# JohnGBaker/ptmcmc

Hardware: AMD Instinct MI355X
Metric: ladder-wide MH steps/sec (D=32 Gaussian, 1024 temps) (higher is better)
Workload: dtype f64

## Files before the change

ptmcmc_amd/csrc/ptm_decide.hpp:

```cpp
#pragma once
#include "ptm_kernels.hpp"

namespace ptm {

constexpr int MSG_HDR = 2;
constexpr int ROW_EXTRA = 4;

__device__ __forceinline__ double* claim_row(double* buf, int cap, int RD, int* err) {
  const int slot = atomicAdd(reinterpret_cast<int*>(buf), 1);
  if (slot >= cap) { atomicOr(err, 4); return nullptr; }
  return buf + MSG_HDR + (size_t)slot * RD;
}

struct Decide {
  int DP, Nt, r0, nloc, W, Nc, ms;
  int w_off;
  uint64_t seed, step;
  double thresh;
  const double* beta;
  const double* ll_below;
  const double* ll_above;
  int H;
  const double* ll_all;
  const double* lp_all;
// ... 680 lines not shown
    d2_t v[NQ];
    const int msrc = lane < nmv ? gs[lane] : 0;
    const int dme = lane < nmv ? gd[lane] : -3;
    const double sl = dme >= 0 ? llc[p.r0 + dme / p.W] : p.ll[msrc];
    const double sp = p.lp_is_const ? p.lp_const : p.lp[msrc];
    for (int hc = 0; hc < DPm; hc += 32) {
      const int colh = col + hc;
#pragma unroll
      for (int q = 0; q < NQ; ++q) {
        const int j = GR * q + g;
        v[q] = *reinterpret_cast<const d2_t*>(p.x + (size_t)(j < nmv ? gs[j] : 0) * DPm + colh);
      }
      asm volatile("s_waitcnt vmcnt(0)" ::: "memory");
      __syncthreads();
#pragma unroll
      for (int q = 0; q < NQ; ++q) {
        const int j = GR * q + g;
        const int d = j < nmv ? gd[j] : -3;
        if (d != -3 && act) {
          double* dstp;
          if (d >= 0) dstp = p.x + (size_t)d * DPm;
          else if (d <= HIST_DST) {
            const int c = HIST_DST - d;
            dstp = p.hist.x + hist_slot(p.hist, 1 + (long long)(p.nhist[c] / (unsigned int)p.add_every_n), c) * DPm;
          } else if (d <= MAP_DST) {
            dstp = p.map.x + (size_t)(MAP_DST - d) * DPm;
          } else { const int e = -d - 4; dstp = ((e & 1) ? p.send_down : p.send_up) + MSG_HDR + (size_t)(e >> 1) * RD; }
          *reinterpret_cast<d2_t*>(dstp + colh) = v[q];
        }
      }
    }
    if (lane < nmv) {
      const int d = gd[lane];
      if (d >= 0) { p.ll[d] = sl; if (!p.lp_is_const) p.lp[d] = sp; }
      else if (d <= HIST_DST) {
        const int c = HIST_DST - d;
        const long long hrow = 1 + (long long)(p.nhist[c] / (unsigned int)p.add_every_n);
        hist_scalars(p.hist, hist_slot(p.hist, hrow, c), hrow, sl, sp, p.naccept[c], p.ntries[c], p.last_type[c],
                     evb ? gb[lane] : beta[p.r0 + c / p.W]);
      } else if (d <= MAP_DST) {
        const int c = MAP_DST - d;
        const double t = (evb ? gb[lane] : beta[p.r0 + c / p.W]) * sl;
        p.map.lpost[c] = sp + t; p.map.ll[c] = sl; p.map.lp[c] = sp;
      } else if (d != -3) {
        const int e = -d - 4;
        double* row = ((e & 1) ? p.send_down : p.send_up) + MSG_HDR + (size_t)(e >> 1) * RD;
        row[DPm] = sl; row[DPm + 1] = sp; row[DPm + 2] = (double)w; row[DPm + 3] = 0.0;
      }
    }
    return;
  }
  const int DP = p.DP;
  if (p.hist.rungs) {
    for (int j = lane; j < nl; j += DECIDE_THREADS) {
      const int k = list[j];
      if (alive[k] != 1) continue;
      const int i = cand[k];
      const int hs = hist_mid_src(i);
      if (hs < 0) continue;
      const int c = (i - p.r0) * p.W + w;
      const long long hrow = 1 + (long long)(p.nhist[c] / (unsigned int)p.add_every_n);
      const size_t o = hist_slot(p.hist, hrow, c);
      for (int d = 0; d < DP; ++d) p.hist.x[o * DP + d] = p.x[(size_t)hs * DP + d];
      hist_scalars(p.hist, o, hrow, p.ll[hs], p.lp[hs], p.naccept[c], p.ntries[c], p.last_type[c], evb ? bklo[k] : beta[i]);
    }
    __syncthreads();
  }
  if (p.map.rungs) {
    for (int j = lane; j < nl; j += DECIDE_THREADS) {
      const int k = list[j];
      if (alive[k] != 1) continue;
      const int i = cand[k];
      const double bmid = evb ? bklo[k] : beta[i];
      const int cs = map_mid_src(i, bmid);
      if (cs < 0) continue;
      const int c = (i - p.r0) * p.W + w;
      const double t = bmid * p.ll[cs];
      p.map.lpost[c] = p.lp[cs] + t; p.map.ll[c] = p.ll[cs]; p.map.lp[c] = p.lp[cs];
      for (int d = 0; d < DP; ++d) p.map.x[(size_t)c * DP + d] = p.x[(size_t)cs * DP + d];
    }
    __syncthreads();
  }
  for (int j = lane; j < nl; j += DECIDE_THREADS) {
    const int k = list[j];
    if (alive[k] != 1) continue;
    const int i = cand[k];
    const int rtop = (PTM_ALIVE_RUNG(i + 1) && alive[first[i + 1]] == 1) ? i : i + 1;
    for (int r = i; r <= rtop; ++r) {
      if (r < p.r0 || r >= r1 || perm[r] == r) continue;
      const int to = inv[r];
      const bool departs = to < p.r0 || to >= r1;
      bool head = departs;
      if (!departs) {
        head = true;
        int cc = perm[r], guard = 0;
        while (cc != r) {
          if (cc < p.r0 || cc >= r1 || cc < r || ++guard > Nt) { head = false; break; }
          cc = perm[cc];
        }
      }
      if (!head) continue;
      double* X = p.x;
      const int c0 = (r - p.r0) * p.W + w;
      if (departs) {
        double* sb = (to >= r1) ? p.send_up : p.send_down;
        if (!sb) continue;
        double* row = claim_row(sb, p.row_cap, DP + ROW_EXTRA, p.err);
        if (row) {
          for (int d = 0; d < DP; ++d) row[d] = X[(size_t)c0 * DP + d];
          row[DP] = p.ll[c0];
          row[DP + 1] = p.lp[c0];
          row[DP + 2] = (double)w;
          row[DP + 3] = 0.0;
        }
      }
      if (p.rowof) {
        const unsigned short carry = p.rowof[c0];
        int cur = r;
        for (int guard = 0; guard <= Nt; ++guard) {
          const int src = perm[cur];
          const int cc = (cur - p.r0) * p.W + w;
          if (src == r) { p.rowof[cc] = carry; break; }
          if (src < p.r0 || src >= r1) break;
          p.rowof[cc] = p.rowof[(src - p.r0) * p.W + w];
          cur = src;
        }
      }
      for (int el = p.rowof ? DP : 0; el < DP + 2; ++el) {
        auto at = [&](int c) -> double* { return el < DP ? X + (size_t)c * DP + el : (el == DP ? p.ll + c : p.lp + c); };
        const double carry = *at(c0);
        int cur = r;
        for (int guard = 0; guard <= Nt; ++guard) {
          const int src = perm[cur];
          const int cc = (cur - p.r0) * p.W + w;
          if (src == r) { *at(cc) = carry; break; }
          if (src < p.r0 || src >= r1) break;
          const int cs = (src - p.r0) * p.W + w;
          *at(cc) = *at(cs);
          cur = src;
        }
      }
    }
  }
  if (lane == 0) p.mv_n[w] = 0;
#undef PTM_ALIVE_RUNG
}

template <int DECIDE_THREADS, bool CUT = false>
__global__ __launch_bounds__(DECIDE_THREADS) void decide_kernel(const Decide p) {
  extern __shared__ __attribute__((aligned(16))) unsigned char smem[];
  decide_body<DECIDE_THREADS, CUT>(p, smem, xcd_walker(blockIdx.x, p.W), p.step, p.swap_log);
}

inline size_t decide_lds_bytes(int Nt, int ms, int WN, bool evolve, bool evb, bool cut = false) {
  if (cut) return decide_lds_bytes(Nt, ms, WN, evolve, true) + (size_t)2 * Nt * 8;
  const bool al = decide_aliased(ms, WN, evolve);
  const size_t msp = (size_t)((ms + 3) & ~3), WNp = (size_t)((WN + 3) & ~3);
  return (size_t)WN * 8 + (size_t)((Nt + 3) & ~3) * 2 + (size_t)((ms + 1) & ~1) * 4 * 2 + 16 + (al ? 0 : 2 * WNp * 2) + 2 * msp * 2 +
         (size_t)((ms + 7) & ~7) * 2 + (al ? 0 : (size_t)2 * MVCAP * 4) + 32 +
         (evolve ? ((size_t)Nt + 2 * ((Nt + 31) / 32) + 2 + 4 * msp) * 8 + 4 * msp * 2 + ((ms + 7) & ~7) : 0) +
         (evb ? ((size_t)(Nt > MVCAP ? Nt : MVCAP) + 5 * msp) * 8 : 0);
}


}
```

ptmcmc_amd/csrc/ptm_engine.hip:

```cpp
#include <hip/hip_runtime.h>

#include <algorithm>
#include <cmath>
#include <cstddef>
#include <cstdarg>
#include <cstdio>
#include <cstring>
#include <functional>
#include <memory>
#include <string>
#include <vector>

#include "../../include/ptm_engine.h"
#include "ptm_aux_kernels.hpp"
#include "ptm_devlike_kernels.hpp"
#include "ptm_ess_kernels.hpp"
#include "ptm_launch.hpp"
#include "ptm_shard_rccl.hpp"

using namespace ptm;

static thread_local std::string g_err;
static int fail(int code, const char* fmt, ...) {
  char buf[512];
// ... 1009 lines not shown
                                 "history_capacity that holds every row of the run");
  if (e->pcb) return fail(PTM_ERR_INVALID, "host-side proposals are set (ptm_set_proposal_callback): they replace every device proposal");
  if (!(q->snooker >= 0 && q->snooker <= 1) || !(q->gamma_one_frac >= 0 && q->gamma_one_frac <= 1) || !(q->reduce_gamma > 0) ||
      !(q->ignore_frac >= 0 && q->ignore_frac < 1) || n_init_extra < 0 || (n_init_extra > 0 && !init_rows))
    return fail(PTM_ERR_INVALID, "differential evolution: snooker and gamma_one_frac in [0, 1], reduce_gamma > 0, ignore_frac in [0, 1), init rows given");
  int rc;
  if (n_init_extra > 0) {
    const size_t Nc = e->Nc, D = e->D, DP = e->DP;
    std::vector<double> img((size_t)n_init_extra * Nc * DP, 0.0);
    for (size_t k = 0; k < (size_t)n_init_extra; ++k)
      for (size_t c = 0; c < Nc; ++c)
        for (size_t d = 0; d < D; ++d) img[(k * Nc + c) * DP + host_row_pos(DP, d)] = init_rows[(k * Nc + c) * D + d];
    if ((rc = dalloc(&e->de_init, img.size()))) return rc;
    HIPCHK(hipMemcpy(e->de_init, img.data(), img.size() * 8, hipMemcpyHostToDevice));
  }
  if (!e->de_hast && ((rc = dalloc(&e->de_hast, (size_t)e->Nc)) || (rc = dalloc(&e->de_type, (size_t)e->Nc)))) return rc;
  e->de = *q;
  e->de_init_extra = n_init_extra;
  e->de_on = true;
  return PTM_OK;
}

extern "C" int ptm_set_proposal_rung(ptm_engine* e, int local_rung, const double* factor, double one_d_frac) {
  SETTLE(e);
  if (!e || !factor) return fail(PTM_ERR_INVALID, "null argument");
  if (!e->have_prop) return fail(PTM_ERR_INVALID, "set all proposals first (ptm_set_proposals)");
  if (local_rung < 0 || local_rung >= e->nloc) return fail(PTM_ERR_INVALID, "rung out of the shard");
  const int D = e->D, DP = e->DP, kind = e->prop_kind == KIND_DIAG ? PTM_PROP_DIAG : (e->prop_kind == KIND_LOWER ? PTM_PROP_LOWER : PTM_PROP_DENSE);
  std::vector<double> packed((size_t)e->prop_stride, 0.0);
  if (kind == PTM_PROP_DIAG) {
    for (int d = 0; d < D; ++d) packed[d] = factor[d];
  } else {
    for (int i = 0; i < D; ++i)
      for (int j = 0; j < D; ++j) {
        if (kind == PTM_PROP_LOWER && j > i && factor[(size_t)i * D + j] != 0.0)
          return fail(PTM_ERR_INVALID, "PTM_PROP_LOWER factor has a non-zero above the diagonal");
        packed[(size_t)j * DP + i] = factor[(size_t)i * D + j];
      }
  }
  int rc;
  if ((rc = upload(e->prop + (size_t)local_rung * e->prop_stride, packed.data(), packed.size(), e->stream))) return rc;
  if (DP == 32) {
    std::vector<double> tiles(16 * 64, 0.0);
    for (int t = 0; t < 16; ++t) {
      const int rt = t & 1, sl = (t >> 1) & 3, hb = t >> 3;
      for (int k = 0; k < 4; ++k)
        for (int i = 0; i < 16; ++i) {
          const int row = 16 * rt + i, col = 16 * hb + 4 * k + sl;
          if (row < D && col < D)
            tiles[(size_t)t * 64 + 16 * k + i] = kind == PTM_PROP_DIAG ? (row == col ? factor[row] : 0.0) : factor[(size_t)row * D + col];
        }
    }
    if ((rc = upload(e->prop_tiles + (size_t)local_rung * 16 * 64, tiles.data(), tiles.size(), e->stream))) return rc;
  }
  if (DP == 64 || DP == 128) {
    const int NT = DP / 16, ntile = NT * NT * 4;
    std::vector<double> tiles((size_t)ntile * 64, 0.0);
    for (int t = 0; t < ntile; ++t) {
      const int rt = t % NT, sl = (t / NT) & 3, hb = t / (4 * NT);
      for (int k = 0; k < 4; ++k)
        for (int i = 0; i < 16; ++i) {
          const int row = 16 * rt + i, col = 16 * hb + 4 * k + sl;
          if (row < D && col < D)
            tiles[(size_t)t * 64 + 16 * k + i] = kind == PTM_PROP_DIAG ? (row == col ? factor[row] : 0.0) : factor[(size_t)row * D + col];
        }
    }
    if ((rc = upload(e->prop_tiles + (size_t)local_rung * ntile * 64, tiles.data(), tiles.size(), e->stream))) return rc;
  }
  if (one_d_frac >= 0) {
    if (one_d_frac > 1) return fail(PTM_ERR_INVALID, "oneDfrac must be in [0,1]");
    if ((rc = upload(e->onedfrac + local_rung, &one_d_frac, 1, e->stream))) return rc;
    if (one_d_frac > 0) e->any_oned = 1;
  }
  return PTM_OK;
}

static Dev make_dev(ptm_engine* e, bool labelled = false) {
  Dev p;
  memset(&p, 0, sizeof p);
  p.D = e->D; p.DP = e->DP; p.Nt = e->Nt; p.r0 = e->r0; p.nloc = e->nloc; p.W = e->W; p.Nc = e->Nc; p.w_off = e->cfg.walker_begin;
  p.seed = e->cfg.seed; p.step = e->step; p.add_every_n = e->cfg.add_every_n; p.min_prior = e->cfg.min_prior;
  p.has_bounds = e->has_bounds; p.origin_valid = e->origin_valid; p.bounds_box = e->bounds_box;
  p.blo = e->blo; p.bhi = e->bhi; p.bmin = e->bmin; p.bmax = e->bmax;
  p.all_uniform = e->all_uniform; p.lprior_const = e->lprior_const;
  p.ptype = e->ptype; p.plo = e->plo; p.phi = e->phi; p.pcoef = e->pcoef;
  p.P2 = e->P2; p.mean = e->mean; p.has_mean = e->has_mean; p.like0 = e->like0;
  p.beta = e->beta; p.prop = e->prop; p.prop_tiles = e->prop_tiles; p.P2_tiles = e->P2_tiles; p.box_row = e->box_row; p.onedfrac = e->onedfrac; p.prop_stride = e->prop_stride; p.any_oned = e->any_oned;
  p.mix_K = e->mix_K; p.mix = e->mix;
  p.de_on = e->de_on ? 1 : 0; p.de_init_extra = e->de_init_extra; p.de_init = e->de_init; p.de_hast = e->de_hast; p.de_type = e->de_type;
  p.de_snooker = e->de.snooker; p.de_gamma_one = e->de.gamma_one_frac; p.de_gamma_div = e->de.reduce_gamma; p.de_ignore = e->de.ignore_frac;
  p.de_gamma_std = e->de_on ? 1.68 / std::sqrt((double)e->D) / e->de.reduce_gamma : 0.0;
  p.betaC = e->betaC; p.beta_add = e->beta_add; p.beta_w = e->beta_w;
  p.x = labelled ? e->xdev : xrows(e); p.ll = e->ll; p.lp = e->lp;
  p.ntries = e->ntries; p.naccept = e->naccept; p.last_type = e->last_type; p.nhist = e->nhist;
  p.touch = e->touch; p.err = e->err;
  p.hist = e->hist;
  p.map = e->map;
  p.c_begin = 0; p.c_end = e->Nc;
  p.host_prop = e->pcb ? 1 : 0; p.hastings = e->hastings; p.htype = e->htype; p.hvalid = e->hvalid; p.acc_out = e->acc_out;
  return p;
}

static AdaArgs make_ada(const ptm_engine* e) {
  AdaArgs a;
  memset(&a, 0, sizeof a);
  if (!e->ada_on) return a;
  const size_t L = (size_t)e->ada.K + e->ada.K_inner, Nc = e->Nc;
  a.K = e->ada.K; a.nested = e->ada.nested; a.Ki = e->ada.K_inner; a.rate = e->ada.rate; a.rate_in = e->ada.rate_inner;
  a.leaf = e->ada_leaf; a.w = e->ada_dbl; a.th = e->ada_dbl + L * Nc; a.bits = e->ada_int; a.cnt = e->ada_int + 2 * Nc;
  return a;
}

static inline bool user_like(const ptm_engine* e) { return e->cb != nullptr || e->dfn != nullptr; }

static SweepSel sweep_sel(const ptm_engine* e) {
  SweepSel s;
  s.kind = e->prop_kind == PTM_PROP_DIAG ? KIND_DIAG : (e->prop_kind == PTM_PROP_LOWER ? KIND_LOWER : KIND_DENSE);
  s.uni = (e->W % 64) == 0;
  s.host_prop = e->pcb != nullptr;
  if (s.host_prop) s.kind = KIND_DIAG;
  s.ada = e->ada_on && !s.host_prop;
  s.plain = !e->has_bounds && e->all_uniform && !e->has_mean && !e->any_oned && !user_like(e) && e->mix_K == 0 && !s.ada && !e->betaC && !s.host_prop;
  s.simple = s.uni && s.plain;
  s.lean_ev = s.uni && e->betaC && !e->has_bounds && e->all_uniform && !e->has_mean && !e->any_oned && !user_like(e) && e->mix_K == 0 && !s.ada && !s.host_prop &&
              !e->hist.rungs && !e->map.rungs;
  s.callback = user_like(e);
  s.de = e->de_on;
  return s;
}

static bool lean_ev_sweeps(const ptm_engine* e) {
  static const bool forced = [] { const char* v = getenv("PTM_FORCE_VALU"); return v && *v && *v != '0'; }();
  return e->DP == 32 && !forced && sweep_sel(e).lean_ev;
}

static int flush_nhist(ptm_engine* e) {
  if (!e->nhist_pending) return PTM_OK;
  hipLaunchKernelGGL(nhist_flush_kernel, dim3((unsigned)(((size_t)e->Nc + 255) / 256)), dim3(256), 0, e->stream, e->nhist, (size_t)e->Nc, e->nhist_pending);
  HIPCHK(hipGetLastError());
  e->nhist_pending = 0;
  return PTM_OK;
}

static bool compact_applies(const ptm_engine* e, const SweepSel& sel) {
  static const bool compact_ok = [] { const char* v = getenv("PTM_COMPACT"); return !(v && *v == '0'); }();
  const bool gen1 = sel.uni && !sel.callback && !sel.host_prop && !sel.de && !sel.ada && e->all_uniform && (!e->has_bounds || e->bounds_box);
  return compact_ok && e->DP == 32 && (sel.simple || gen1) && !e->hist.rungs && !e->map.rungs && !getenv("PTM_FORCE_VALU") &&
         e->W >= 1024 && e->nloc <= 4096;
}
static bool row_labels_apply(const ptm_engine* e) {
  static const bool labels_ok = [] { const char* v = getenv("PTM_ROW_LABELS"); return !(v && *v == '0'); }();
  return labels_ok && e->nloc == e->Nt && !e->shard && e->W <= 65536 && e->Nt > 1 && compact_applies(e, sweep_sel(e));
}
static void flush_rows(ptm_engine* e) {
  e->rows_labelled = false;
  hipLaunchKernelGGL(restore_rows_kernel, dim3(e->W), dim3(256), (size_t)4 * e->nloc, e->stream, e->xdev, e->rowof, e->W, e->nloc, e->DP);
}

static int ensure_betaC(ptm_engine* e);
static int callback_host_part(ptm_engine* e) {
  const size_t Nc = e->Nc, DP = e->DP;
  HIPCHK(copy_unless_shared(e->h_xprop.data(), e->xprop, Nc * DP * 8 + Nc, hipMemcpyDeviceToHost, e->stream));
  HIPCHK(hipStreamSynchronize(e->stream));
  if (e->prior_cb) {
    std::vector<double> hll(Nc), hlp(Nc), hbeta(Nc), out;
    HIPCHK(hipMemcpy(hll.data(), e->ll, Nc * 8, hipMemcpyDeviceToHost));
    HIPCHK(hipMemcpy(hlp.data(), e->lp, Nc * 8, hipMemcpyDeviceToHost));
    { int rc2 = ensure_betaC(e); if (rc2) return rc2; }
    if (e->betaC) HIPCHK(hipMemcpy(hbeta.data(), e->betaC, Nc * 8, hipMemcpyDeviceToHost));
    std::vector<size_t> vp;
    for (size_t c = 0; c < Nc; ++c)
      if (e->h_gate[c] & 1) vp.push_back(c);
    int rcp = call_user_prior(e, e->h_xprop, vp, out);
    if (rcp) return rcp;
    std::vector<double> lpn(Nc, -__builtin_inf());
    for (size_t k = 0; k < vp.size(); ++k) {
      const size_t c = vp[k];
      const double beta = e->betaC ? hbeta[c] : e->h_beta[e->r0 + c / e->W];
      const double bl = beta * hll[c];
      const double cur_lpost = hlp[c] + bl;
      const double oldlprior = cur_lpost - bl;
      const double nl = out[k];
      lpn[c] = nl;
      const bool want = nl > -1e200 || nl - oldlprior > e->cfg.min_prior;
      e->h_gate[c] = (unsigned char)(1 | (want ? 2 : 0));
    }
    HIPCHK(hipMemcpyAsync(e->lprior_new, lpn.data(), Nc * 8, hipMemcpyHostToDevice, e->stream));
    HIPCHK(copy_unless_shared(e->gate, e->h_gate, Nc, hipMemcpyHostToDevice, e->stream));
    HIPCHK(hipStreamSynchronize(e->stream));
  }
  std::vector<size_t> pick;
  for (size_t c = 0; c < Nc; ++c)
    if (e->h_gate[c] & 2) pick.push_back(c);
  int rc = call_user(e, e->h_xprop, pick, e->h_llbatch);
  if (rc) return rc;
  for (size_t k = 0; k < pick.size(); ++k) e->h_llnew[pick[k]] = e->h_llbatch[k];
  HIPCHK(copy_unless_shared(e->llike_new, e->h_llnew.data(), Nc * 8, hipMemcpyHostToDevice, e->stream));
  return PTM_OK;
}

static int devlike_eval(ptm_engine* e, const unsigned char* gate, int gmask, int gval, const double* xsel, const double* xrest, double* dst,
                        unsigned char* gate_out, const double* lprior, bool best) {
  const int n = e->Nc, D = e->D;
  const int nchunk = (n + DL_CHUNK - 1) / DL_CHUNK;
  hipLaunchKernelGGL(devlike_count_kernel, dim3(nchunk), dim3(DL_CHUNK), 0, e->stream, n, gate, gmask, gval, e->dl_chunks);
  HIPCHK(hipGetLastError());
#define PTM_DL_PACK(N) case N: hipLaunchKernelGGL((devlike_pack_kernel<N>), dim3(nchunk), dim3(DL_CHUNK), 0, e->stream, n, D, nchunk, gate, gmask, gval, \
                                                  (const int*)e->dl_chunks, xsel, xrest, e->dl_x, e->dl_rows, e->dl_count); break;
  switch (e->DP) {
    PTM_DL_PACK(4) PTM_DL_PACK(8) PTM_DL_PACK(16) PTM_DL_PACK(32) PTM_DL_PACK(64) PTM_DL_PACK(128) PTM_DL_PACK(256) PTM_DL_PACK(512) PTM_DL_PACK(1024)
    default: return fail(PTM_ERR_UNSUPPORTED, "dim > 1024 is not built");
  }
#undef PTM_DL_PACK
  HIPCHK(hipGetLastError());
  if (!xrest) {
    const size_t tot = (size_t)n * D;
    hipLaunchKernelGGL(devlike_fill_kernel, dim3((unsigned)((tot + 255) / 256)), dim3(256), 0, e->stream, n, D, (const int32_t*)e->dl_count, e->dl_x);
    HIPCHK(hipGetLastError());
  }
  e->dfn(e->dfn_user, (void*)e->stream, n, D, e->dl_x, e->dl_count, e->dl_ll);
  hipLaunchKernelGGL(devlike_scatter_kernel, dim3(1), dim3(DL_SCATTER_THREADS), 0, e->stream, D, (const int32_t*)e->dl_count, (const int*)e->dl_rows,
                     (const double*)e->dl_ll, dst, gate_out, lprior, (const double*)e->dl_x, best ? e->dl_best : nullptr);
  HIPCHK(hipGetLastError());
  return PTM_OK;
}

static int devlike_reset_best(ptm_engine* e) {
  if (!e->dl_best) return PTM_OK;
  std::vector<double> b((size_t)e->D + 1, 0.0);
  b[0] = -__builtin_inf();
  return upload(e->dl_best, b.data(), b.size(), e->stream);
}

extern "C" int ptm_set_target_device(ptm_engine* e, ptm_loglike_device_fn fn, void* user, double* x_batch_dev, double* llike_batch_dev) {
  if (!e || !fn) return fail(PTM_ERR_INVALID, "null argument");
  SETTLE(e);
  NO_BATCH(e, "ptm_set_target_device");
  if (e->prior_cb) return fail(PTM_ERR_UNSUPPORTED, "a host-evaluated prior with a device likelihood is not built (ptm_set_prior_callback)");
  if (e->pcb) return fail(PTM_ERR_UNSUPPORTED, "host-side proposals with a device likelihood are not built (ptm_set_proposal_callback)");
  if (e->nloc != e->Nt) return fail(PTM_ERR_UNSUPPORTED, "a device likelihood on a rung shard is not built: split such a population by walkers");
  const size_t Nc = e->Nc, D = e->D, DP = e->DP;
  int rc;
  if (!e->dl_count &&
      ((rc = dalloc(&e->dl_count, 1)) || (rc = dalloc(&e->dl_rows, Nc)) || (rc = dalloc(&e->dl_chunks, (Nc + DL_CHUNK - 1) / DL_CHUNK)) ||
       (rc = dalloc(&e->dl_xprop, Nc * DP)) || (rc = dalloc(&e->dl_gate, Nc)) || (rc = dalloc(&e->dl_lprior_new, Nc)) ||
       (rc = dalloc(&e->dl_llike_new, Nc)) || (rc = dalloc(&e->dl_best, D + 1))))
    return rc;
  if (x_batch_dev) {
    if (e->dl_own_x && e->dl_x) { HIPCHK(hipStreamSynchronize(e->stream)); (void)hipFree(e->dl_x); }
    e->dl_x = x_batch_dev; e->dl_own_x = false;
  } else if (!e->dl_own_x) {
    e->dl_x = nullptr;
    if ((rc = dalloc(&e->dl_x, Nc * D))) return rc;
    e->dl_own_x = true;
  }
  if (llike_batch_dev) {
    if (e->dl_own_ll && e->dl_ll) { HIPCHK(hipStreamSynchronize(e->stream)); (void)hipFree(e->dl_ll); }
    e->dl_ll = llike_batch_dev; e->dl_own_ll = false;
  } else if (!e->dl_own_ll) {
    e->dl_ll = nullptr;
    if ((rc = dalloc(&e->dl_ll, Nc))) return rc;
    e->dl_own_ll = true;
  }
  HIPCHK(hipMemsetAsync(e->dl_gate, 0, Nc, e->stream));
  if ((rc = devlike_reset_best(e))) return rc;
  e->dfn = fn; e->dfn_user = user;
  e->cb = nullptr;
  e->have_target = 1;
  return PTM_OK;
}

extern "C" int ptm_target_device_rows(ptm_engine* e) {
  if (!e) return fail(PTM_ERR_INVALID, "null engine");
  return e->Nc;
}

extern "C" int ptm_get_best_evaluated(ptm_engine* e, double* lpost, double* x) {
  if (!e || !lpost) return fail(PTM_ERR_INVALID, "null argument");
  SETTLE(e);
  NO_BATCH(e, "ptm_get_best_evaluated");
  if (!e->dl_best) return fail(PTM_ERR_INVALID, "no device likelihood set (ptm_set_target_device)");
  std::vector<double> b((size_t)e->D + 1);
  HIPCHK(hipMemcpyAsync(b.data(), e->dl_best, b.size() * 8, hipMemcpyDeviceToHost, e->stream));
  HIPCHK(hipStreamSynchronize(e->stream));
  *lpost = b[0];
  if (x) memcpy(x, b.data() + 1, (size_t)e->D * 8);
  return PTM_OK;
}

static int devlike_debug(ptm_engine* e, const double* X, int n, double* llike) {
  const size_t Nc = e->Nc, D = e->D;
  std::vector<double> rows(Nc * D);
  for (size_t k0 = 0; k0 < (size_t)n; k0 += Nc) {
    const size_t m = std::min(Nc, (size_t)n - k0);
    for (size_t k = 0; k < Nc; ++k) memcpy(&rows[k * D], X + (k0 + (k < m ? k : 0)) * D, D * 8);
    const int32_t cnt = (int32_t)m;
    HIPCHK(hipMemcpyAsync(e->dl_x, rows.data(), Nc * D * 8, hipMemcpyHostToDevice, e->stream));
    HIPCHK(hipMemcpyAsync(e->dl_count, &cnt, 4, hipMemcpyHostToDevice, e->stream));
    e->dfn(e->dfn_user, (void*)e->stream, (int)Nc, (int)D, e->dl_x, e->dl_count, e->dl_ll);
    HIPCHK(hipMemcpyAsync(llike + k0, e->dl_ll, m * 8, hipMemcpyDeviceToHost, e->stream));
    HIPCHK(hipStreamSynchronize(e->stream));
  }
  return PTM_OK;
}

#define NO_DEVLIKE(e, name) do { if ((e) && (e)->dfn) return fail(PTM_ERR_UNSUPPORTED, name " with a device likelihood is not built (rung-sharded steps)"); } while (0)
// ... 43 lines not shown
      case 16: return launch_sweep_16(q, sel, e->stream, ada);
      case 32: return launch_sweep_32(q, sel, e->stream, ada);
      case 64: return launch_sweep_64(q, sel, e->stream, ada);
      case 128: return launch_sweep_128(q, sel, e->stream, ada);
      case 256: return launch_sweep_256(q, sel, e->stream, ada);
      case 512: return launch_sweep_512(q, sel, e->stream, ada);
      case 1024: return launch_sweep_1024(q, sel, e->stream, ada);
    }
    return hipErrorInvalidValue;
  };

  size_t npick = 0;
  if (e->pcb) {
    const size_t Nc = e->Nc, D = e->D, DP = e->DP;
    HIPCHK(hipMemcpyAsync(e->h_rows.data(), xrows(e), Nc * DP * 8, hipMemcpyDeviceToHost, e->stream));
    HIPCHK(hipMemcpyAsync(e->h_touch.data(), e->touch, Nc, hipMemcpyDeviceToHost, e->stream));
    HIPCHK(hipStreamSynchronize(e->stream));
    e->p_pick.clear();
    for (size_t c = 0; c < Nc; ++c)
      if (!e->h_touch[c]) e->p_pick.push_back(c);
    npick = e->p_pick.size();
    e->p_xcur.resize(npick * D); e->p_xprop.assign(npick * D, 0.0); e->p_hast.assign(npick, 0.0);
    e->p_rung.resize(npick); e->p_walker.resize(npick); e->p_type.assign(npick, 0); e->p_valid.assign(npick, 1);
    for (size_t k = 0; k < npick; ++k) {
      const size_t c = e->p_pick[k];
      for (size_t d = 0; d < D; ++d) e->p_xcur[k * D + d] = e->h_rows[c * DP + host_row_pos(DP, d)];
      e->p_rung[k] = e->r0 + (int)(c / e->W); e->p_walker[k] = e->cfg.walker_begin + (int)(c % e->W);
    }
    if (npick)
      e->pcb(e->pcb_user, (int)npick, (int)D, e->p_xcur.data(), e->p_rung.data(), e->p_walker.data(), e->step, e->p_xprop.data(),
             e->p_hast.data(), e->p_type.data(), e->p_valid.data());
    for (size_t k = 0; k < npick; ++k) {
      const size_t c = e->p_pick[k];
      for (size_t d = 0; d < DP; ++d) e->h_xprop[c * DP + d] = 0.0;
      for (size_t d = 0; d < D; ++d) e->h_xprop[c * DP + host_row_pos(DP, d)] = e->p_xprop[k * D + d];
      e->h_hast[c] = e->p_hast[k]; e->h_type[c] = e->p_type[k]; e->h_valid[c] = e->p_valid[k] ? 1 : 0;
    }
    HIPCHK(copy_unless_shared(e->xprop, e->h_xprop.data(), Nc * DP * 8, hipMemcpyHostToDevice, e->stream));
    HIPCHK(copy_unless_shared(e->hastings, e->h_hast.data(), Nc * 8, hipMemcpyHostToDevice, e->stream));
    HIPCHK(copy_unless_shared(e->htype, e->h_type.data(), Nc * 4, hipMemcpyHostToDevice, e->stream));
    HIPCHK(copy_unless_shared(e->hvalid, e->h_valid.data(), Nc, hipMemcpyHostToDevice, e->stream));
    p.xprop = e->xprop; p.lprior_new = e->lprior_new; p.gate = e->gate; p.llike_new = e->llike_new;
  }
  if (e->dfn) {
    p.xprop = e->dl_xprop; p.lprior_new = e->dl_lprior_new; p.gate = e->dl_gate; p.llike_new = e->dl_llike_new;
    p.mode = 1;
    HIPCHK(launch(p));
    { const int rc = devlike_eval(e, e->dl_gate, 2, 2, e->dl_xprop, xrows(e), e->dl_llike_new, nullptr, e->dl_lprior_new, true); if (rc) return rc; }
    p.mode = 2;
    HIPCHK(launch(p));
  } else if (!e->cb) {
    HIPCHK(launch(p));
  } else {
    const size_t Nc = e->Nc, DP = e->DP;
    p.xprop = e->xprop; p.lprior_new = e->lprior_new; p.gate = e->gate; p.llike_new = e->llike_new;
    p.mode = 1;
    HIPCHK(launch(p));
    { const int rc = callback_host_part(e); if (rc) return rc; }
    p.mode = 2;
    HIPCHK(launch(p));
  }
  if (e->pcb && e->pres && npick) {
    HIPCHK(copy_unless_shared(e->h_acc.data(), e->acc_out, (size_t)e->Nc, hipMemcpyDeviceToHost, e->stream));
    HIPCHK(hipStreamSynchronize(e->stream));
    e->p_acc.resize(npick);
    for (size_t k = 0; k < npick; ++k) e->p_acc[k] = e->h_acc[e->p_pick[k]] == 1 ? 1 : 0;
    e->pres(e->pcb_user, (int)npick, e->p_rung.data(), e->p_walker.data(), e->p_acc.data());
  }
  if (ev1) HIPCHK(hipEventRecord(ev1, e->stream));
  if (last) close_step();
  return PTM_OK;
}

static int fold_swap_log(ptm_engine* e) {
  if (!e->log_pending) return PTM_OK;
  const int first = ((e->log_head - e->log_pending) % PTM_LOG_RING + PTM_LOG_RING) % PTM_LOG_RING;
  if (e->Nt > 1) {
    hipLaunchKernelGGL(fold_swap_log_kernel, dim3(e->W), dim3(256), (size_t)2 * (e->Nt - 1) * sizeof(int), e->stream, e->swap_log, e->swap_cnt,
                       e->W, e->ms, e->Nt, e->r0, e->r0 + e->nloc, first, e->log_pending);
    HIPCHK(hipGetLastError());
  }
  e->log_pending = 0;
  return PTM_OK;
}

static int launch_beta_transpose(ptm_engine* e) {
  e->betaC_stale = false;
  if (e->nloc != e->Nt) {
    hipLaunchKernelGGL(beta_local_kernel, dim3((unsigned)(((size_t)e->Nc + 255) / 256)), dim3(256), 0, e->stream, e->beta_w, e->betaC, e->W, e->Nt, e->r0, e->nloc);
    HIPCHK(hipGetLastError());
    return PTM_OK;
  }
  hipLaunchKernelGGL(beta_transpose_kernel, dim3((e->Nt + 31) / 32, (e->W + 31) / 32), dim3(256), 0, e->stream, e->beta_w, e->betaC, e->W, e->Nt);
  HIPCHK(hipGetLastError());
  return PTM_OK;
}
static int ensure_betaC(ptm_engine* e) {
  if (!e->betaC_stale) return PTM_OK;
  e->betaC_stale = false;
  return launch_beta_transpose(e);
}

static Decide make_decide(ptm_engine* e, const double* ll_below, const double* ll_above, int H, double* send_up, double* send_down,
                          const double* ll_all = nullptr, const double* lp_all = nullptr, bool labels = false) {
  Decide p;
  memset(&p, 0, sizeof p);
  p.rowof = labels ? e->rowof : nullptr;
  p.ll_all = ll_all; p.lp_all = lp_all;
  p.shard_ends = e->shard_ends; p.nshards = e->nshards; p.halo_nominal = e->halo_nominal;
  p.redo_flag = e->redo_flag; p.redo_count = e->redo_flag ? e->redo_flag + e->W : nullptr;
  p.DP = e->DP; p.Nt = e->Nt; p.r0 = e->r0; p.nloc = e->nloc; p.W = e->W; p.Nc = e->Nc; p.ms = e->ms; p.w_off = e->cfg.walker_begin;
  p.seed = e->cfg.seed; p.step = e->step; p.thresh = e->thresh;
  p.beta = e->beta; p.ll_below = ll_below; p.ll_above = ll_above; p.H = ll_above ? H : 0; p.x = labels ? e->xdev : xrows(e); p.ll = e->ll; p.lp = e->lp;
  p.touch = e->touch; p.arr_below = e->arr_below; p.arr_above = e->arr_above;
  p.swap_log = e->swap_log + (size_t)e->log_head * e->W * e->ms; p.send_up = send_up; p.send_down = send_down; p.row_cap = e->row_cap; p.err = e->err;
  p.mv_src = e->mv_src; p.mv_dst = e->mv_dst; p.mv_n = e->mv_n;
  p.hist = e->hist; p.add_every_n = e->cfg.add_every_n; p.nhist = e->nhist;
  p.naccept = e->naccept; p.ntries = e->ntries; p.last_type = e->last_type;
  p.map = e->map;
  p.evolve_rate = e->evolve_rate; p.evolve_cut = e->evolve_cut; p.beta_w = e->beta_w; p.beta_add = e->beta_add;
  p.lp_is_const = e->lp_is_const ? 1 : 0; p.lp_const = e->lprior_const;
  static const bool direct_all = [] { const char* v = getenv("PTM_BETA_DIRECT"); return v && *v == '1'; }();
  const bool beta_direct = e->evolve_rate > 0 && (e->W <= 64 || direct_all);
  p.betaC_direct = beta_direct ? e->betaC : nullptr;
  return p;
}

static int launch_decide(ptm_engine* e, const double* ll_below, const double* ll_above, int H, double* send_up, double* send_down,
                         const double* ll_all = nullptr, const double* lp_all = nullptr, bool redo = false, bool labels = false) {
  if (labels && !e->rowof) {
    int rc = dalloc(&e->rowof, (size_t)e->Nc);
    if (rc) return rc;
    hipLaunchKernelGGL(identity_rows_kernel, dim3((unsigned)(((size_t)e->Nc + 255) / 256)), dim3(256), 0, e->stream, e->rowof, e->W, (size_t)e->Nc);
    HIPCHK(hipGetLastError());
  }
  Decide p = make_decide(e, ll_below, ll_above, H, send_up, send_down, ll_all, lp_all, labels);
  if (labels) { e->rows_labelled = true; e->label_step = true; }
  p.redo_only = redo ? 1 : 0;
  if (!redo && e->log_pending >= PTM_LOG_RING) { int rc = fold_swap_log(e); if (rc) return rc; }
  if (redo) {
    const int slot = (e->log_head + PTM_LOG_RING - 1) % PTM_LOG_RING;
    p.swap_log = e->swap_log + (size_t)slot * e->W * e->ms;
  }
  const bool beta_direct = p.betaC_direct != nullptr;
  e->touched = true;
  const int WN = ll_all ? e->Nt : e->nloc + (ll_below ? 1 : 0) + p.H;
  const bool evb = e->evolve_rate > 0 && e->beta_add;
  const bool cut = e->evolve_rate > 0 && e->evolve_cut >= 0;
  const size_t lds = decide_lds_bytes(e->Nt, e->ms, WN, e->evolve_rate > 0, evb, cut);
  if (lds > 160 * 1024) return fail(PTM_ERR_UNSUPPORTED, "ladder too long for the LDS-resident exchange kernel (%zu B)", lds);
  if (e->ms >= 65535) return fail(PTM_ERR_UNSUPPORTED, "more than 65534 exchange candidates per step (the exchange kernel numbers them in 16 bits)");
  const int per_pick = (e->nloc == e->Nt ? 2 : 4) + (e->hist.rungs ? 1 : 0) + (e->map.rungs ? 1 : 0);
  const bool wide = (double)e->ms * WN / e->Nt > 96.0 || evb || cut || (e->W <= 256 && per_pick * e->ms > 64);
  if (lds > 64 * 1024) {
    HIPCHK(hipFuncSetAttribute((const void*)decide_kernel<64>, hipFuncAttributeMaxDynamicSharedMemorySize, (int)lds));
    HIPCHK(hipFuncSetAttribute((const void*)decide_kernel<256>, hipFuncAttributeMaxDynamicSharedMemorySize, (int)lds));
  }
  if (send_up && !redo) HIPCHK(hipMemsetAsync(send_up, 0, 16, e->stream));
  if (send_down && !redo) HIPCHK(hipMemsetAsync(send_down, 0, 16, e->stream));
  if (cut) {
    if (lds > 64 * 1024) HIPCHK(hipFuncSetAttribute((const void*)decide_kernel<256, true>, hipFuncAttributeMaxDynamicSharedMemorySize, (int)lds));
    hipLaunchKernelGGL((decide_kernel<256, true>), dim3(e->W), dim3(256), lds, e->stream, p);
  } else if (wide) hipLaunchKernelGGL(decide_kernel<256>, dim3(e->W), dim3(256), lds, e->stream, p);
  else hipLaunchKernelGGL(decide_kernel<64>, dim3(e->W), dim3(64), lds, e->stream, p);
  HIPCHK(hipGetLastError());
  if (!redo) {
    e->log_head = (e->log_head + 1) % PTM_LOG_RING;
    ++e->log_pending;
  }
  if (e->evolve_rate > 0 && !beta_direct) {
    if (lean_ev_sweeps(e)) e->betaC_stale = true;
    else { e->betaC_stale = false; int rc = launch_beta_transpose(e); if (rc) return rc; }
  }
  if (wide) return PTM_OK;
  if (per_pick * e->ms <= 64 || labels) return PTM_OK;
  Move m;
  m.DP = e->DP; m.W = e->W; m.row_cap = e->row_cap; m.x = xrows(e); m.ll = e->ll; m.lp = e->lp; m.send_up = send_up; m.send_down = send_down;
  m.mv_src = e->mv_src; m.mv_dst = e->mv_dst; m.mv_n = e->mv_n; m.err = e->err;
  m.hist = e->hist; m.add_every_n = e->cfg.add_every_n; m.nhist = e->nhist;
  m.naccept = e->naccept; m.ntries = e->ntries; m.last_type = e->last_type;
  m.map = e->map; m.beta = e->beta; m.r0 = e->r0;
  const dim3 mgrid((unsigned)((e->W + 63) / 64));
  if (e->hist.rungs || e->map.rungs) hipLaunchKernelGGL((move_kernel<MVCAP, 1, true>), mgrid, dim3(64), 0, e->stream, m);
  else hipLaunchKernelGGL((move_kernel<MVCAP, 1, false>), mgrid, dim3(64), 0, e->stream, m);
  HIPCHK(hipGetLastError());
  return PTM_OK;
}

static int launch_install(ptm_engine* e, const double* recv_below, const double* recv_above) {
  if (!recv_below && !recv_above) return PTM_OK;
  Install q;
  q.DP = e->DP; q.W = e->W; q.row_cap = e->row_cap; q.x = xrows(e); q.ll = e->ll; q.lp = e->lp;
  q.recv_below = recv_below; q.recv_above = recv_above; q.arr_below = e->arr_below; q.arr_above = e->arr_above; q.err = e->err;
  e->touched = true;
  hipLaunchKernelGGL(install_kernel, dim3((e->row_cap + 15) / 16, 2), dim3(256), 0, e->stream, q);
  HIPCHK(hipGetLastError());
  return PTM_OK;
}

static int ready(ptm_engine* e) {
  if (!e) return fail(PTM_ERR_INVALID, "null engine");
  if (!e->have_target) return fail(PTM_ERR_INVALID, "no target set (ptm_set_target_gaussian)");
  if (!e->have_ladder) return fail(PTM_ERR_INVALID, "no ladder set (ptm_set_ladder)");
  if (!e->have_prop) return fail(PTM_ERR_INVALID, "no proposals set (ptm_set_proposals)");
  if (!e->have_state) return fail(PTM_ERR_INVALID, "no states set (ptm_set_states / ptm_init_from_prior)");
  return PTM_OK;
}

static int check_lp_const(ptm_engine* e) {
  e->lp_is_const = false;
  if (!e->all_uniform || e->prior_cb) return PTM_OK;
  std::vector<double> lp((size_t)e->Nc);
  HIPCHK(hipStreamSynchronize(e->stream));
  HIPCHK(hipMemcpy(lp.data(), e->lp, lp.size() * 8, hipMemcpyDeviceToHost));
  for (double v : lp)
    if (!(v == e->lprior_const)) return PTM_OK;
  e->lp_is_const = true;
  return PTM_OK;
}
static int reset_counters(ptm_engine* e) {
  const size_t Nc = e->Nc;
  std::vector<int> one(Nc, 1), m1(Nc, -1);
  std::vector<unsigned int> z(Nc, 0u);
  int rc;
  if ((rc = upload(e->ntries, one.data(), Nc, e->stream)) || (rc = upload(e->naccept, one.data(), Nc, e->stream)) ||
      (rc = upload(e->last_type, m1.data(), Nc, e->stream)) ||
      (rc = upload(e->nhist, z.data(), Nc, e->stream)))
    return rc;
  e->nhist_pending = 0; e->compact_step = false; e->touched = false;
  HIPCHK(hipMemsetAsync(e->touch, 0, Nc, e->stream));
  HIPCHK(hipMemsetAsync(e->arr_below, 0xFF, (size_t)e->W * 4, e->stream));
  HIPCHK(hipMemsetAsync(e->arr_above, 0xFF, (size_t)e->W * 4, e->stream));
  e->step = 0;
  if (e->map.rungs) {
    if (!e->have_ladder) return fail(PTM_ERR_INVALID, "set the ladder before the states when tracking the MAP (ptm_set_ladder)");
    hipLaunchKernelGGL(map_init_kernel, dim3((e->map.MC + 255) / 256), dim3(256), 0, e->stream, e->map, e->DP, e->W, e->r0, e->beta, xrows(e), e->ll,
                       e->lp);
    HIPCHK(hipGetLastError());
  }
  if (e->hist.rungs) {
    HIPCHK(hipMemsetAsync(e->hist.meta, 0xFF, (size_t)e->hist.cap * e->hist.HC * sizeof(int4), e->stream));
    if (e->hist.beta && !e->have_ladder) return fail(PTM_ERR_INVALID, "set the ladder before the states (ptm_set_ladder)");
    hipLaunchKernelGGL(hist_init_kernel, dim3((e->hist.HC + 255) / 256), dim3(256), 0, e->stream, e->hist, e->DP, xrows(e), e->ll, e->lp,
                       e->naccept, e->ntries, e->last_type, e->beta, e->betaC, e->W, e->r0);
    HIPCHK(hipGetLastError());
  }
  return PTM_OK;
}

static int run_eval(ptm_engine* e, int n, double* x, int* valid, double* lp, double* ll, int eval_like) {
  Dev p = make_dev(e);
  switch (e->DP) {
    case 4: HIPCHK(launch_eval_4(p, n, x, valid, lp, ll, eval_like, e->stream)); break;
    case 8: HIPCHK(launch_eval_8(p, n, x, valid, lp, ll, eval_like, e->stream)); break;
    case 16: HIPCHK(launch_eval_16(p, n, x, valid, lp, ll, eval_like, e->stream)); break;
    case 32: HIPCHK(launch_eval_32(p, n, x, valid, lp, ll, eval_like, e->stream)); break;
    case 64: HIPCHK(launch_eval_64(p, n, x, valid, lp, ll, eval_like, e->stream)); break;
    case 128: HIPCHK(launch_eval_128(p, n, x, valid, lp, ll, eval_like, e->stream)); break;
    case 256: HIPCHK(launch_eval_256(p, n, x, valid, lp, ll, eval_like, e->stream)); break;
    case 512: HIPCHK(launch_eval_512(p, n, x, valid, lp, ll, eval_like, e->stream)); break;
    case 1024: HIPCHK(launch_eval_1024(p, n, x, valid, lp, ll, eval_like, e->stream)); break;
    default: return fail(PTM_ERR_UNSUPPORTED, "dim > 1024 is not built");
  }
  return PTM_OK;
}

static inline size_t host_row_pos(size_t DP, size_t d) { return (DP == 32 || DP == 64 || DP == 128) ? 8 * ((d >> 2) >> 1) + 2 * (d & 3) + ((d >> 2) & 1) : d; }
static std::vector<double> pad_rows(const double* X, size_t n, size_t D, size_t DP) {
  std::vector<double> r(n * DP, 0.0);
  for (size_t c = 0; c < n; ++c)
    for (size_t d = 0; d < D; ++d) r[c * DP + host_row_pos(DP, d)] = X[c * D + d];
  return r;
}
static void unpad_rows(const double* r, size_t n, size_t D, size_t DP, double* X) {
  for (size_t c = 0; c < n; ++c)
    for (size_t d = 0; d < D; ++d) X[c * D + d] = r[c * DP + host_row_pos(DP, d)];
}
static void unpad_rows(const std::vector<double>& r, size_t n, size_t D, size_t DP, double* X) { unpad_rows(r.data(), n, D, DP, X); }

extern "C" int ptm_set_states(ptm_engine* e, const double* X, const double* llike) {
  SETTLE(e);
  NO_BATCH(e, "ptm_set_states");
  if (!e || !X) return fail(PTM_ERR_INVALID, "null argument");
  if (!e->have_target && !llike) return fail(PTM_ERR_INVALID, "set the target first (or pass llike)");
  const size_t Nc = e->Nc, D = e->D, DP = e->DP;
  const std::vector<double> rows = pad_rows(X, Nc, D, DP);
  int rc;
  if ((rc = upload(xrows(e), rows.data(), Nc * DP, e->stream))) return rc;
  if (llike && (rc = upload(e->ll, llike, Nc, e->stream))) return rc;
  if ((rc = run_eval(e, (int)Nc, xrows(e), nullptr, e->lp, e->ll, (llike || user_like(e)) ? 0 : 1))) return rc;
  if (e->dfn) {
    if ((rc = devlike_reset_best(e))) return rc;
    if (!llike && (rc = devlike_eval(e, nullptr, 0, 0, xrows(e), xrows(e), e->ll, nullptr, e->lp, true))) return rc;
  }
  if (e->cb && !llike) {
    HIPCHK(hipStreamSynchronize(e->stream));
    HIPCHK(hipMemcpy(e->h_xprop.data(), xrows(e), Nc * DP * 8, hipMemcpyDeviceToHost));
    std::vector<size_t> all(Nc);
    for (size_t c = 0; c < Nc; ++c) all[c] = c;
    if ((rc = call_user(e, e->h_xprop, all, e->h_llbatch))) return rc;
    if ((rc = upload(e->ll, e->h_llbatch.data(), Nc, e->stream))) return rc;
  }
  if (e->prior_cb) {
    if (!e->cb) return fail(PTM_ERR_UNSUPPORTED, "a host-evaluated prior needs the host-callback likelihood (ptm_set_target_callback)");
    HIPCHK(hipStreamSynchronize(e->stream));
    HIPCHK(hipMemcpy(e->h_xprop.data(), xrows(e), Nc * DP * 8, hipMemcpyDeviceToHost));
// ... 1556 lines not shown
```

Measured before the change: 9.934 billion.

## Add lean specialised exchange-decision kernel for the common unsharded row-label path

```diff
diff --git a/ptmcmc_amd/csrc/ptm_decide.hpp b/ptmcmc_amd/csrc/ptm_decide.hpp
--- a/ptmcmc_amd/csrc/ptm_decide.hpp
+++ b/ptmcmc_amd/csrc/ptm_decide.hpp
@@ -856,6 +856,118 @@
   decide_body<DECIDE_THREADS, CUT>(p, smem, xcd_walker(blockIdx.x, p.W), p.step, p.swap_log);
 }
 
+template <int DECIDE_THREADS>
+__device__ __forceinline__ void decide_lean_body(const Decide& p, unsigned char* smem, const int w, const uint64_t step, int* const swap_log) {
+  const int lane = threadIdx.x;
+  const int Nt = p.Nt, ms = p.ms, W = p.W;
+  const int NONE = 0xffff;
+  const int msp = (ms + 3) & ~3;
+  double* llc = reinterpret_cast<double*>(smem);
+  double* dbt = llc + 2 * msp;
+  uint32_t* ua = reinterpret_cast<uint32_t*>(dbt + msp);
+  int* cand = reinterpret_cast<int*>(ua + msp);
+  unsigned short* first = reinterpret_cast<unsigned short*>(cand + msp);
+  unsigned short* src = first + ((Nt + 3) & ~3);
+  unsigned short* lab = src + 2 * msp;
+  unsigned char* alive = reinterpret_cast<unsigned char*>(lab + 2 * msp);
+  unsigned char* accf = alive + ((ms + 7) & ~7);
+  cdp beta = as_c(p.beta);
+
+  for (int i = lane; i < ((Nt + 3) & ~3) / 2; i += DECIDE_THREADS) reinterpret_cast<uint32_t*>(first)[i] = 0xffffffffu;
+  __syncthreads();
+  const uint64_t try_below = u01_below_bound(p.thresh);
+  for (int k = lane; k < ms; k += DECIDE_THREADS) {
+    const u32x4 o = draw_block(p.seed, TAG_PT, (uint32_t)(w + p.w_off), step, (uint32_t)k);
+    int n = -2;
+    if ((uint64_t)o.v0 < try_below) n = u01_times(o.v1, Nt - 1);
+    cand[k] = n;
+    ua[k] = o.v2;
+    alive[k] = 0;
+    accf[k] = 0;
+    if (n >= 0) lds_min_u16(first, n, (unsigned int)k);
+  }
+  __syncthreads();
+  for (int k = lane; k < ms; k += DECIDE_THREADS) {
+    const int n = cand[k];
+    if (n < 0 || first[n] != k) continue;
+    if (n > 0 && first[n - 1] != NONE) continue;
+    bool a = true;
+    for (int m = n;; ++m) {
+      alive[first[m]] = a ? 1 : 0;
+      if (m + 1 > Nt - 2 || first[m + 1] == NONE) break;
+      a = !(a && first[m] < first[m + 1]);
+    }
+  }
+  __syncthreads();
+#define PTM_ALIVE_RUNG(r) ((r) >= 0 && (r) <= Nt - 2 && first[(r)] != NONE && alive[first[(r)]])
+  for (int k = lane; k < ms; k += DECIDE_THREADS) {
+    if (!alive[k]) continue;
+    const int n = cand[k];
+    const bool top = !PTM_ALIVE_RUNG(n + 1);
+    const size_t c = (size_t)n * W + w;
+    const double a = p.ll[c];
+    const unsigned short la = p.rowof[c];
+    const double b0 = beta[n], b1 = beta[n + 1];
+    double b = 0.0;
+    unsigned short lb = 0;
+    if (top) { b = p.ll[c + W]; lb = p.rowof[c + W]; }
+    p.touch[c] = (unsigned char)(1 + (PTM_ALIVE_RUNG(n - 1) ? 1 : 0));
+    if (top) p.touch[c + W] = 1;
+    llc[2 * k] = a; lab[2 * k] = la; src[2 * k] = (unsigned short)(2 * k);
+    if (top) { llc[2 * k + 1] = b; lab[2 * k + 1] = lb; src[2 * k + 1] = (unsigned short)(2 * k + 1); }
+    dbt[k] = b1 - b0;
+  }
+  __syncthreads();
+  for (int k0 = lane; k0 < ms; k0 += DECIDE_THREADS) {
+    if (!alive[k0]) continue;
+    int i = cand[k0];
+    if (PTM_ALIVE_RUNG(i + 1)) continue;
+    int k = k0, sh = 2 * k0 + 1;
+    double vhi = llc[sh];
+    unsigned short phi = (unsigned short)sh;
+    for (;; --i) {
+      const int sl = 2 * k;
+      const double vlo = llc[sl];
+      double lla = vlo;
+      if (!(lla > -1e200)) lla = -1e200;
+      double llb = vhi;
+      if (!(llb > -1e200)) llb = -1e200;
+      const double logH = -dbt[k] * (llb - lla);
+      bool acc = true;
+      if (logH < 0) acc = dlog_u01(ua[k]) < logH;
+      llc[sh] = acc ? vlo : vhi;
+      src[sh] = acc ? (unsigned short)sl : phi;
+      if (acc) accf[k] = 1; else { vhi = vlo; phi = (unsigned short)sl; }
+      sh = sl;
+      if (!PTM_ALIVE_RUNG(i - 1)) break;
+      k = first[i - 1];
+    }
+    llc[sh] = vhi;
+    src[sh] = phi;
+  }
+  __syncthreads();
+  for (int k = lane; k < ms; k += DECIDE_THREADS) {
+    swap_log[(size_t)w * ms + k] = alive[k] ? (cand[k] | (accf[k] ? 0x40000000 : 0)) : -2;
+    if (!alive[k]) continue;
+    const int n = cand[k];
+    const size_t c = (size_t)n * W + w;
+    if (src[2 * k] != 2 * k) { p.rowof[c] = lab[src[2 * k]]; p.ll[c] = llc[2 * k]; }
+    if (!PTM_ALIVE_RUNG(n + 1) && src[2 * k + 1] != 2 * k + 1) { p.rowof[c + W] = lab[src[2 * k + 1]]; p.ll[c + W] = llc[2 * k + 1]; }
+  }
+#undef PTM_ALIVE_RUNG
+}
+
+template <int DECIDE_THREADS>
+__global__ __launch_bounds__(DECIDE_THREADS) void decide_lean_kernel(const Decide p) {
+  extern __shared__ __attribute__((aligned(16))) unsigned char smem[];
+  decide_lean_body<DECIDE_THREADS>(p, smem, xcd_walker(blockIdx.x, p.W), p.step, p.swap_log);
+}
+
+inline size_t decide_lean_lds_bytes(int Nt, int ms) {
+  const size_t msp = (size_t)((ms + 3) & ~3);
+  return 2 * msp * 8 + msp * 8 + msp * 4 * 2 + (size_t)((Nt + 3) & ~3) * 2 + 2 * msp * 2 * 2 + (size_t)((ms + 7) & ~7) * 2;
+}
+
 inline size_t decide_lds_bytes(int Nt, int ms, int WN, bool evolve, bool evb, bool cut = false) {
   if (cut) return decide_lds_bytes(Nt, ms, WN, evolve, true) + (size_t)2 * Nt * 8;
   const bool al = decide_aliased(ms, WN, evolve);
diff --git a/ptmcmc_amd/csrc/ptm_engine.hip b/ptmcmc_amd/csrc/ptm_engine.hip
--- a/ptmcmc_amd/csrc/ptm_engine.hip
+++ b/ptmcmc_amd/csrc/ptm_engine.hip
@@ -1185,6 +1185,12 @@
   static const bool labels_ok = [] { const char* v = getenv("PTM_ROW_LABELS"); return !(v && *v == '0'); }();
   return labels_ok && e->nloc == e->Nt && !e->shard && e->W <= 65536 && e->Nt > 1 && compact_applies(e, sweep_sel(e));
 }
+static bool decide_lean_applies(const ptm_engine* e, const Decide& p) {
+  static const bool lean_ok = [] { const char* v = getenv("PTM_DECIDE_LEAN"); return !(v && *v == '0'); }();
+  return lean_ok && p.rowof && e->r0 == 0 && e->nloc == e->Nt && e->Nt > 1 && !(e->evolve_rate > 0) && !e->hist.rungs && !e->map.rungs &&
+         !p.beta_add && !p.send_up && !p.send_down && !p.ll_all && !p.ll_below && !p.ll_above && !p.redo_only && p.lp_is_const &&
+         e->ms <= 32767 && decide_lean_lds_bytes(e->Nt, e->ms) <= 64 * 1024;
+}
 static void flush_rows(ptm_engine* e) {
   e->rows_labelled = false;
   hipLaunchKernelGGL(restore_rows_kernel, dim3(e->W), dim3(256), (size_t)4 * e->nloc, e->stream, e->xdev, e->rowof, e->W, e->nloc, e->DP);
@@ -1534,6 +1540,15 @@
   if (e->ms >= 65535) return fail(PTM_ERR_UNSUPPORTED, "more than 65534 exchange candidates per step (the exchange kernel numbers them in 16 bits)");
   const int per_pick = (e->nloc == e->Nt ? 2 : 4) + (e->hist.rungs ? 1 : 0) + (e->map.rungs ? 1 : 0);
   const bool wide = (double)e->ms * WN / e->Nt > 96.0 || evb || cut || (e->W <= 256 && per_pick * e->ms > 64);
+  if (decide_lean_applies(e, p)) {
+    const size_t llds = decide_lean_lds_bytes(e->Nt, e->ms);
+    if (wide) hipLaunchKernelGGL(decide_lean_kernel<256>, dim3(e->W), dim3(256), llds, e->stream, p);
+    else hipLaunchKernelGGL(decide_lean_kernel<64>, dim3(e->W), dim3(64), llds, e->stream, p);
+    HIPCHK(hipGetLastError());
+    e->log_head = (e->log_head + 1) % PTM_LOG_RING;
+    ++e->log_pending;
+    return PTM_OK;
+  }
   if (lds > 64 * 1024) {
     HIPCHK(hipFuncSetAttribute((const void*)decide_kernel<64>, hipFuncAttributeMaxDynamicSharedMemorySize, (int)lds));
     HIPCHK(hipFuncSetAttribute((const void*)decide_kernel<256>, hipFuncAttributeMaxDynamicSharedMemorySize, (int)lds));
```

Result: no change. 9.989 billion (median of 6 runs) (+0.6%).
